# mengxuyiGit/LGM

Measured on AMD Instinct MI355X. Metric: Mpixels/s fwd+bwd Gaussian raster (256^2, 100k gauss, 6 views), higher is better.
Workload: dtype f32

## Files before the change

include/lgm_common.h:

```cpp
#ifndef LGM_COMMON_H
#define LGM_COMMON_H
#include <stddef.h>
#ifdef __cplusplus
extern "C" {
#endif

#define LGM_OK 0
#define LGM_E_INVALID -1
#define LGM_E_WORKSPACE -2
#define LGM_E_HIP -3

const char *lgm_last_error(void);

int lgm_abi_version(void);

typedef struct lgm_profiler lgm_profiler;
lgm_profiler *lgm_profiler_create(void);
int lgm_profiler_summary(lgm_profiler *p, char *buf, size_t len);
int lgm_profiler_reset(lgm_profiler *p);
void lgm_profiler_destroy(lgm_profiler *p);

typedef struct lgm_diag {
    lgm_profiler *profiler;
    unsigned long long *render_counters;
    int det_limit_log2;
} lgm_diag;

#ifdef __cplusplus
}
#endif
#endif
```

lgm_amd/_native.py:

```python
from __future__ import annotations

import contextlib
import ctypes
import os

import torch

LIB_PATH = os.environ.get("LGM_AMD_LIB") or os.path.join(os.path.dirname(os.path.abspath(__file__)), "_lib",
                                                          "liblgm_amd.so")

_c_int, _c_ll, _c_float, _c_size, _vp = ctypes.c_int, ctypes.c_longlong, ctypes.c_float, ctypes.c_size_t, ctypes.c_void_p
_c_double = ctypes.c_double

SIGNATURES = {
    "lgm_abi_version": (_c_int, []),
    "lgm_last_error": (ctypes.c_char_p, []),
    "lgm_render_workspace_size": (_c_size, [_c_int, _c_int, _c_int, _c_int, _c_int, _c_ll]),
    "lgm_render_workspace_size_opts": (_c_size, [_c_int, _c_int, _c_int, _c_int, _c_int, _c_ll, _c_int]),
    "lgm_render_count_pairs": (_c_int, [_c_int, _c_int, _c_int, _c_int, _c_int, _vp, _vp, _vp, _c_float, _c_float,
                                        _c_float, _vp, _c_size, _vp, _vp, _vp]),
    "lgm_render_forward": (_c_int, [_c_int, _c_int, _c_int, _c_int, _c_int, _vp, _vp, _vp, _vp, _c_float, _c_float,
                                    _c_float, _vp, _vp, _vp, _vp, _vp, _c_size, _c_ll, _vp, _c_int, _vp, _vp]),
    "lgm_render_backward": (_c_int, [_c_int, _c_int, _c_int, _c_int, _c_int, _vp, _vp, _vp, _vp, _c_float, _c_float,
                                     _c_float, _vp, _vp, _vp, _vp, _vp, _vp, _c_size, _c_ll, _c_int, _vp, _vp]),
# ... 1 lines not shown
                                  _vp, _vp]),
    "lgm_attn_backward": (_c_int, [_c_int, _c_int, _c_int, _c_int, _c_int, _c_float, _vp, _vp, _vp, _c_ll, _vp, _vp,
                                   _vp, _vp, _vp, _vp, _c_ll, _vp, _c_size, _vp, _vp]),
    "lgm_attn_workspace_size": (_c_size, [_c_int, _c_int, _c_int, _c_int, _c_int]),
    "lgm_mva_workspace_size": (_c_size, [_c_int, _c_int, _c_int, _c_int, _c_int]),
    "lgm_mva_norm_tokens": (_c_int, [_c_int, _c_int, _c_int, _c_int, _c_int, _c_int, _c_int, _c_float, _vp, _vp, _vp,
                                     _vp, _vp, _vp, _vp, _c_size, _vp, _vp]),
    "lgm_mva_tokens_out": (_c_int, [_c_int, _c_int, _c_int, _c_int, _c_int, _c_int, _c_int, _vp, _vp, _c_float, _vp,
                                    _vp, _vp]),
    "lgm_mva_backward_workspace_size": (_c_size, [_c_int, _c_int, _c_int, _c_int, _c_int]),
    "lgm_mva_tokens_out_backward": (_c_int, [_c_int, _c_int, _c_int, _c_int, _c_int, _c_int, _c_int, _vp, _c_float, _vp,
                                             _vp, _vp, _vp]),
    "lgm_mva_norm_tokens_backward": (_c_int, [_c_int, _c_int, _c_int, _c_int, _c_int, _c_int, _c_int, _vp, _vp, _vp,
                                              _vp, _vp, _vp, _vp, _vp, _vp, _vp, _c_size, _vp, _vp]),
    "lgm_render_forward_loss": (_c_int, [_c_int, _c_int, _c_int, _c_int, _c_int, _vp, _vp, _vp, _vp, _c_float,
                                         _c_float, _c_float, _vp, _vp, _vp, _vp, _vp, _vp, _vp, _c_size, _c_ll, _c_int,
                                         _vp, _vp]),
    "lgm_render_backward_loss": (_c_int, [_c_int, _c_int, _c_int, _c_int, _c_int, _vp, _vp, _vp, _vp, _c_float,
                                          _c_float, _c_float, _vp, _vp, _vp, _vp, _vp, _vp, _vp, _c_size, _c_ll,
                                          _c_int, _vp, _vp]),
    "lgm_render_tile_lists": (_c_int, [_c_int, _c_int, _c_int, _c_int, _c_int, _vp, _c_size, _c_ll, _vp, _vp, _vp,
                                       _vp]),
    "lgm_render_pixel_state": (_c_int, [_c_int, _c_int, _c_int, _c_int, _c_int, _vp, _c_size, _c_ll, _vp, _vp, _vp]),
    "lgm_render_records": (_c_int, [_c_int, _c_int, _c_int, _c_int, _c_int, _vp, _c_size, _c_ll, _vp, _vp, _vp, _vp]),
    "lgm_render_needle_flags": (_c_int, [_c_ll, _vp, _vp, _vp]),
    "lgm_render_det_flush_limit_log2": (_c_int, [_c_int, _c_int, _c_int]),
    "lgm_gaussian_head_forward": (_c_int, [_c_int, _c_int, _c_int, _c_int, _c_int, _vp, _vp, _vp, _vp, _vp, _vp,
                                           _c_size, _vp, _vp]),
    "lgm_gaussian_head_workspace_size": (_c_size, [_c_int, _c_int, _c_int, _c_int]),
    "lgm_gaussian_head_backward": (_c_int, [_c_int, _c_int, _c_int, _c_int, _c_int, _vp, _vp, _vp, _vp, _vp, _vp, _vp,
                                            _vp, _vp, _c_size, _vp, _vp]),
    "lgm_linear_wgrad_workspace_size": (_c_size, [_c_int, _c_int, _c_int, _c_int]),
    "lgm_linear_wgrad": (_c_int, [_c_int, _c_int, _c_int, _c_int, _vp, _c_ll, _vp, _c_ll, _vp, _vp, _vp, _c_size,
                                  _vp, _vp]),
    "lgm_conv_wgrad_workspace_size": (_c_size, [_c_int, _c_int, _c_int, _c_int, _c_int, _c_int, _c_int]),
    "lgm_conv_wgrad": (_c_int, [_c_int, _c_int, _c_int, _c_int, _c_int, _c_int, _c_int, _vp, _vp, _vp, _vp, _vp, _c_size,
                                _vp, _vp]),
    "lgm_conv_forward_workspace_size": (_c_size, [_c_int, _c_int, _c_int, _c_int, _c_int, _c_int]),
    "lgm_conv_forward": (_c_int, [_c_int, _c_int, _c_int, _c_int, _c_int, _c_int, _c_int, _c_int, _vp, _vp, _vp, _c_int,
                                  _vp, _vp, _c_size, _vp, _vp]),
    "lgm_conv_dgrad_workspace_size": (_c_size, [_c_int, _c_int, _c_int, _c_int, _c_int, _c_int]),
    "lgm_conv_dgrad": (_c_int, [_c_int, _c_int, _c_int, _c_int, _c_int, _c_int, _c_int, _c_int, _vp, _vp, _vp, _vp,
                                _c_size, _vp, _vp]),
    "lgm_gn_silu_workspace_size": (_c_size, [_c_int, _c_int, _c_int, _c_int, _c_int]),
    "lgm_gn_silu_forward": (_c_int, [_c_int, _c_int, _c_int, _c_int, _c_int, _c_int, _c_int, _c_float, _c_int, _vp, _vp,
                                     _vp, _vp, _vp, _vp, _vp, _c_size, _vp, _vp]),
    "lgm_gn_silu_backward_workspace_size": (_c_size, [_c_int, _c_int, _c_int, _c_int, _c_int]),
    "lgm_gn_silu_backward": (_c_int, [_c_int, _c_int, _c_int, _c_int, _c_int, _c_int, _c_int, _c_int, _vp, _vp, _vp,
                                      _vp, _vp, _vp, _vp, _vp, _vp, _vp, _c_size, _vp, _vp]),
    "lgm_lpips_dist_workspace_size": (_c_size, [_c_int, _c_int, _c_int, _c_int]),
    "lgm_lpips_dist_forward": (_c_int, [_c_int, _c_int, _c_int, _c_int, _c_int, _c_int, _c_float, _vp, _vp, _vp, _vp,
                                        _vp, _vp, _vp, _c_size, _vp, _vp]),
    "lgm_lpips_dist_backward": (_c_int, [_c_int, _c_int, _c_int, _c_int, _c_int, _c_int, _c_float, _vp, _vp, _vp, _vp,
                                         _vp, _vp, _vp, _vp, _vp, _vp]),
    "lgm_lpips_prep_forward": (_c_int, [_c_int, _c_int, _c_int, _c_int, _vp, _vp, _vp, _vp, _vp, _vp, _vp, _vp]),
    "lgm_lpips_prep_backward": (_c_int, [_c_int, _c_int, _c_int, _c_int, _vp, _vp, _vp, _vp]),
    "lgm_data_cameras": (_c_int, [_c_int, _c_int, _c_int, _vp, _vp, _c_double, _c_double, _c_double, _c_double,
                                  _c_double, _vp, _vp, _vp, _vp, _vp, _vp, _vp]),
    "lgm_data_views": (_c_int, [_c_int, _c_int, _c_int, _c_int, _c_int, _c_int, _c_int, _c_int, _c_int, _vp, _vp, _vp,
                                _vp, _c_double, _vp, _vp, _vp, _vp, _vp]),
    "lgm_optim_workspace_size": (_c_size, [_c_ll]),
    "lgm_optim_grad_norm": (_c_int, [_vp, _c_int, _vp, _c_ll, _c_double, _vp, _c_size, _vp, _vp, _vp]),
    "lgm_optim_adamw": (_c_int, [_vp, _c_int, _vp, _c_ll, _c_ll, _vp, _c_double, _c_double, _c_double, _c_double,
                                 _c_double, _c_double, _vp, _vp]),
    "lgm_optim_scale": (_c_int, [_vp, _c_int, _vp, _c_ll, _vp, _vp, _vp]),
    "lgm_mesh_density_workspace_size": (_c_size, [_c_ll, _c_int, _c_int, _c_int, _c_ll]),
    "lgm_mesh_density_count": (_c_int, [_vp, _c_ll, _c_float, _c_int, _c_int, _c_int, _vp, _vp, _c_float, _vp, _c_size,
                                        _vp, _vp, _vp]),
    "lgm_mesh_density": (_c_int, [_vp, _c_ll, _c_float, _c_int, _c_int, _c_int, _vp, _vp, _c_float, _c_ll, _vp, _vp, _vp,
                                  _c_size, _vp, _vp]),
    "lgm_mesh_extract_workspace_size": (_c_size, [_c_int, _c_int, _c_int]),
    "lgm_mesh_count": (_c_int, [_vp, _c_int, _c_int, _c_int, _c_float, _vp, _c_size, _vp, _vp, _vp]),
    "lgm_mesh_emit": (_c_int, [_vp, _vp, _c_int, _c_int, _c_int, _vp, _vp, _c_float, _vp, _c_size, _c_ll, _c_ll, _vp, _vp,
                               _vp, _c_ll, _c_ll, _vp, _vp]),
    "lgm_profiler_create": (_vp, []),
    "lgm_profiler_summary": (_c_int, [_vp, ctypes.c_char_p, _c_size]),
    "lgm_profiler_reset": (_c_int, [_vp]),
    "lgm_profiler_destroy": (None, [_vp]),
}

_lib = None


ABI_VERSION = 10
DTYPE_CODES = {torch.float32: 0, torch.bfloat16: 1, torch.float16: 2}
RENDER_NO_CULL = 1
RENDER_CLAMP_IMAGE = 2
RENDER_BACKWARD_AGAIN = 4
RENDER_DETERMINISTIC = 16
DATA_U8 = 3
OPTIM_CHUNK = 4096


class NativeError(RuntimeError):
    pass


def lib():
    global _lib
    if _lib is None:
        if not os.path.exists(LIB_PATH):
            raise NativeError(f"lgm_amd native library not built ({LIB_PATH}); run `python -m lgm_amd.build`")
        L = ctypes.CDLL(LIB_PATH)
        for name, (res, args) in SIGNATURES.items():
            fn = getattr(L, name, None)
            if fn is None:
                continue
            fn.restype = res
            fn.argtypes = args
        if L.lgm_abi_version() != ABI_VERSION:
            raise NativeError(f"{LIB_PATH}: ABI {L.lgm_abi_version()} != {ABI_VERSION}; rebuild (python -m lgm_amd.build)")
        _lib = L
    return _lib


def check(rc: int, what: str):
    if rc != 0:
        msg = lib().lgm_last_error()
        raise NativeError(f"{what} failed (rc={rc}): {msg.decode() if msg else ''}")


def ptr(t):
    return None if t is None else ctypes.c_void_p(t.data_ptr())


def stream_of(device) -> ctypes.c_void_p:
    return ctypes.c_void_p(torch.cuda.current_stream(device).cuda_stream)


def require_device_tensor(t: torch.Tensor, name: str):
    if not t.is_cuda:
        raise NativeError(f"{name} must be a GPU tensor: lgm_amd has no CPU path (the reference's rasterizer is "
                          "GPU-only too, core/gs.py:20)")


class _Diag(ctypes.Structure):
    _fields_ = [("profiler", _vp), ("render_counters", _vp), ("det_limit_log2", ctypes.c_int)]


_diag_cur = None


def diag():
    return None if _diag_cur is None else ctypes.byref(_diag_cur)


@contextlib.contextmanager
def diagnostics(profiler=None, render_counters=None, det_limit_log2=0):
    global _diag_cur
    prev = _diag_cur
    d = _Diag(profiler.h if profiler is not None else None,
              render_counters.data_ptr() if render_counters is not None else None, int(det_limit_log2))
    _diag_cur = d
    try:
        yield d
    finally:
        _diag_cur = prev


class KernelProfiler:

    def __init__(self):
        self.h = lib().lgm_profiler_create()
        self._cm = None

    def __enter__(self):
        self._cm = diagnostics(profiler=self)
        self._cm.__enter__()
        return self

    def __exit__(self, *exc):
        cm, self._cm = self._cm, None
        return cm.__exit__(*exc)

    def reset(self):
        lib().lgm_profiler_reset(self.h)

    def summary(self):
        buf = ctypes.create_string_buffer(1 << 16)
        check(lib().lgm_profiler_summary(self.h, buf, len(buf)), "lgm_profiler_summary")
        out = {}
        for line in buf.value.decode().splitlines():
            name, n, ms = line.split()
            out[name] = (int(n), float(ms))
        return out

    def close(self):
        if self.h:
            lib().lgm_profiler_destroy(self.h)
            self.h = None
```

lgm_amd/csrc/common.hip:

```cpp
#include "common.h"

#include <stdarg.h>
#include <string.h>

#include <map>
#include <mutex>
#include <string>
#include <vector>

#include "lgm_attn.h"
#include "lgm_common.h"

struct lgm_profiler {
    struct Rec { const char *name; hipEvent_t a, b; };
    std::mutex mu;
    std::vector<Rec> recs;
    std::vector<hipEvent_t> pool;
    size_t used = 0;
    hipEvent_t get() {
        if (used == pool.size()) {
            hipEvent_t e;
            if (hipEventCreate(&e) != hipSuccess) return nullptr;
            pool.push_back(e);
        }
        return pool[used++];
    }
};

namespace lgm {
static thread_local char g_err[512] = {0};
static thread_local const lgm_diag *g_call_diag = nullptr;
static thread_local const char *g_pending = nullptr;
static thread_local hipEvent_t g_pending_ev = nullptr;

void set_error(const char *fmt, ...) {
    va_list ap;
    va_start(ap, fmt);
    vsnprintf(g_err, sizeof(g_err), fmt, ap);
    va_end(ap);
}
void clear_error() { g_err[0] = 0; }

int check_dtype16(const char *who, int dtype) {
    if (dtype == LGM_ATTN_BF16 || dtype == LGM_ATTN_F16) return LGM_OK;
    set_error("%s: dtype must be bf16 or fp16 (got %d)", who, dtype);
    return LGM_E_INVALID;
}
int check_workspace(const char *who, const void *ws, size_t have, size_t need) {
    if (have >= need && (!need || ws)) return LGM_OK;
    set_error("%s: workspace too small (%zu < %zu bytes)", who, ws ? have : 0, need);
    return LGM_E_WORKSPACE;
}

static thread_local int g_scope_depth = 0;
DiagScope::DiagScope(const lgm_diag *d) {
    if (g_scope_depth++ == 0) g_call_diag = d;
}
DiagScope::~DiagScope() {
    if (--g_scope_depth == 0) {
        g_call_diag = nullptr;
        g_pending_ev = nullptr;
    }
}
const lgm_diag *call_diag() { return g_call_diag; }

static lgm_profiler *call_profiler() { return g_call_diag ? g_call_diag->profiler : nullptr; }

void prof_begin(const char *name, hipStream_t st) {
    lgm_profiler *p = call_profiler();
    if (!p) return;
    std::lock_guard<std::mutex> lk(p->mu);
    g_pending = name;
    g_pending_ev = p->get();
    if (g_pending_ev) (void)hipEventRecord(g_pending_ev, st);
}
void prof_end(hipStream_t st) {
    lgm_profiler *p = call_profiler();
    if (!p || !g_pending_ev) return;
    std::lock_guard<std::mutex> lk(p->mu);
    hipEvent_t b = p->get();
    if (!b) return;
    (void)hipEventRecord(b, st);
    p->recs.push_back({g_pending, g_pending_ev, b});
    g_pending_ev = nullptr;
}
}

extern "C" {
const char *lgm_last_error(void) { return lgm::g_err; }
int lgm_abi_version(void) { return 10; }

lgm_profiler *lgm_profiler_create(void) { return new lgm_profiler(); }
int lgm_profiler_reset(lgm_profiler *p) {
    if (!p) return LGM_E_INVALID;
    std::lock_guard<std::mutex> lk(p->mu);
    p->recs.clear();
    p->used = 0;
    return LGM_OK;
}
int lgm_profiler_summary(lgm_profiler *p, char *buf, size_t len) {
    if (!p || !buf || len == 0) return LGM_E_INVALID;
    std::map<std::string, std::pair<int, double>> agg;
    std::vector<std::string> order;
    for (auto &r : p->recs) {
        if (hipEventSynchronize(r.b) != hipSuccess) {
            lgm::set_error("event sync failed");
            return LGM_E_HIP;
        }
        float ms = 0.f;
        (void)hipEventElapsedTime(&ms, r.a, r.b);
        auto it = agg.find(r.name);
        if (it == agg.end()) {
            order.push_back(r.name);
            agg[r.name] = {1, ms};
        } else {
            it->second.first++;
            it->second.second += ms;
        }
    }
    std::string out;
    char line[256];
    for (auto &n : order) {
        snprintf(line, sizeof(line), "%s %d %.6f\n", n.c_str(), agg[n].first, agg[n].second);
        out += line;
    }
    strncpy(buf, out.c_str(), len - 1);
    buf[len - 1] = 0;
    return LGM_OK;
}
void lgm_profiler_destroy(lgm_profiler *p) {
    if (!p) return;
    for (auto e : p->pool) (void)hipEventDestroy(e);
    delete p;
}
}
```

lgm_amd/csrc/render_bin.hip:

```cpp
#include "render_common.h"

namespace lgm {
namespace {

enum BinMode { COUNT = 0, EMIT_SLOT = 1, EMIT_PACKED = 2 };

template <int CTRL, int ROW_MASK = 0xf>
__device__ __forceinline__ int dpp_src(int old, int v) {
    return __builtin_amdgcn_update_dpp(old, v, CTRL, ROW_MASK, 0xf, false);
}
__device__ __forceinline__ int wave_incl_scan(int x, int ) {
    x += dpp_src<0x111>(0, x);
    x += dpp_src<0x112>(0, x);
    x += dpp_src<0x114>(0, x);
    x += dpp_src<0x118>(0, x);
    x += dpp_src<0x142, 0xa>(0, x);
    x += dpp_src<0x143, 0xc>(0, x);
    return x;
}

constexpr int BIN_THREADS = 512, BIN_G = BIN_THREADS, BIN_ITERS = 3;
constexpr int BIN_HITCAP = BIN_THREADS * 6;
static_assert(BIN_THREADS <= 512, "owner index and tile rank pack into 9 bits each");
static_assert(LDS_HIST_MAX <= 1 << 13, "the tile index of a hit packs into 13 bits");
#ifndef LGM_BIN_WAVES
#define LGM_BIN_WAVES 6
#endif
constexpr int bin_waves(bool stats) { return stats ? 4 : LGM_BIN_WAVES; }

struct BinRec {
    float x, y, kB, k0, k1, dys, mg;
    unsigned c0;
    unsigned cx1;
    unsigned pad_;
    unsigned long long key;
};

__device__ __forceinline__ int wave_incl_max(int v, int ) {
    constexpr int LO = -2147483647 - 1;
    v = max(v, dpp_src<0x111>(LO, v));
    v = max(v, dpp_src<0x112>(LO, v));
    v = max(v, dpp_src<0x114>(LO, v));
    v = max(v, dpp_src<0x118>(LO, v));
    v = max(v, dpp_src<0x142, 0xa>(LO, v));
    v = max(v, dpp_src<0x143, 0xc>(LO, v));
    return v;
}

__device__ void center_order(int gx, int T, int *__restrict__ corder, int *hk) {
    const int gy = (T + gx - 1) / gx, tid = threadIdx.x, w = tid >> 6, lane = tid & 63;
    const int K = min(T, BIN_THREADS);
    const long long maxkey = (long long)(gx - 1) * (gx - 1) + (long long)(gy - 1) * (gy - 1);
    auto key = [&](int t) {
        const int y = t / gx, x = t - y * gx, dx = 2 * x - (gx - 1), dy = 2 * y - (gy - 1);
        return maxkey ? (int)(((long long)dx * dx + (long long)dy * dy) * (K - 1) / maxkey) : 0;
    };
    __syncthreads();
    if (tid < K) hk[tid] = 0;
    __syncthreads();
    for (int t = tid; t < T; t += BIN_THREADS) atomicAdd(&hk[key(t)], 1);
    __syncthreads();
    const int v = tid < K ? hk[tid] : 0;
    const int incl = wave_incl_scan(v, lane);
    if (lane == 63) hk[K + w] = incl;
    __syncthreads();
    int run = incl - v;
    for (int ww = 0; ww < w; ww++) run += hk[K + ww];
    __syncthreads();
    if (tid < K) hk[tid] = run;
    __syncthreads();
    for (int t = tid; t < T; t += BIN_THREADS) corder[atomicAdd(&hk[key(t)], 1)] = t;
}

template <int MODE, bool STATS, bool STAMPS>
__global__ __launch_bounds__(BIN_THREADS) __attribute__((amdgpu_waves_per_eu(bin_waves(STATS)))) void k_bin(
    Dims d, const float *__restrict__ gauss, const float *__restrict__ views, const float *__restrict__ projs,
    float4 *__restrict__ gP, float4 *__restrict__ gQ, uint2 *__restrict__ rects, int *__restrict__ radii_out,
    int *__restrict__ tile_count, const int *__restrict__ tile_start, unsigned long long *__restrict__ pairs,
    long long slot_stride, unsigned long long *__restrict__ misc, float *__restrict__ accum,
    int *__restrict__ corder) {
    extern __shared__ int hist[];
    __shared__ BinRec srec[BIN_THREADS];
    __shared__ int sHead[BIN_THREADS], sExcl[BIN_THREADS];
    __shared__ unsigned sHit[BIN_HITCAP];
    __shared__ int s_nhit;
    __shared__ unsigned long long s_tot[2];
    const int T = d.T, tid = threadIdx.x, w = tid >> 6, lane = tid & 63;
    const int vgroups = (d.V + BIN_ITERS - 1) / BIN_ITERS;
    const int b = blockIdx.y / vgroups, vg0 = (blockIdx.y - b * vgroups) * BIN_ITERS;
    int bv = b * d.V + vg0;
    const bool lds = T <= LDS_HIST_MAX;
    int *hbase = hist + T, *fill = hist + 2 * T;
    int *cur = tile_count + (size_t)bv * T;
    if constexpr (STATS)
        if (tid < 2) s_tot[tid] = 0;
    auto dest = [&](int t, int pos) -> long long {
        return (MODE == EMIT_SLOT ? ((long long)bv * T + t) * slot_stride
                                  : (long long)tile_start[(size_t)bv * T + t]) + pos;
    };
    __shared__ unsigned long long s_ph[4];
    unsigned long long *stamp = nullptr;
    if constexpr (STAMPS) {
        stamp = d.counters + 8 + 8 * (size_t)d.BV * T + 8 * ((size_t)blockIdx.y * gridDim.x + blockIdx.x);
        if (tid == 0) {
            s_ph[0] = s_ph[1] = s_ph[2] = 0;
            stamp[0] = s_ph[3] = __builtin_amdgcn_s_memrealtime();
        }
    }
    auto phase = [&](int k) {
        if constexpr (STAMPS) {
            if (tid == 0) {
                const unsigned long long t = __builtin_amdgcn_s_memrealtime();
                if (k >= 0) s_ph[k] += t - s_ph[3];
                s_ph[3] = t;
            }
        }
    };
    const int i = blockIdx.x * BIN_G + tid;
    float c3[6];
    if (i < d.N) {
        float g[14];
        load_gaussian(gauss + ((size_t)b * d.N + i) * 14, g);
        gaussian_cov3d(g, d.mod, c3);
    }
    for (int it = 0; it < BIN_ITERS; it++) {
    if (vg0 + it >= d.V) break;
    bv = b * d.V + vg0 + it;
    cur = tile_count + (size_t)bv * T;
    if (tid == 0) s_nhit = 0;
    if (lds)
        for (int t = tid; t < T; t += BIN_THREADS) hist[t] = 0;
    Geo o;
    bool vis = false;
    if (i < d.N) {
        const float2 *gp = reinterpret_cast<const float2 *>(gauss + ((size_t)b * d.N + i) * 14);
        const float2 g01 = gp[0], g23 = gp[1];
        const float gm[4] = {g01.x, g01.y, g23.x, g23.y};
        vis = preprocess_view(gm, c3, views + 16 * bv, projs + 16 * bv, d, o);
        if (MODE != COUNT) {
            const size_t k = (size_t)bv * d.N + i;
            if (vis) {
                const float4 rp = rec_p(o.x, o.y, o.A, o.B), rq = rec_q(o.C, o.opacity, o.tau, o.depth);
                gP[k] = rp;
                gQ[k] = rq;
                const bool side = !(d.options & LGM_RENDER_DETERMINISTIC) && rec_needle(rp.z, rp.w, rq.x);
                rects[k] = make_uint2((unsigned)o.x0 | ((unsigned)o.y0 << 16),
                                      (unsigned)o.x1 | ((unsigned)o.y1 << 16) | (side ? 0x80000000u : 0u));
                if (side) {
                    double *sd = reinterpret_cast<double *>(accum + acc_side_offset(d.B, d.V, d.N)) + k * 3;
                    sd[0] = 0.0; sd[1] = 0.0; sd[2] = 0.0;
                }
            } else {
                gP[k] = make_float4(0.f, 0.f, 0.f, 0.f);
                gQ[k] = make_float4(0.f, -INFINITY, -1.f, 0.f);
                rects[k] = make_uint2(0u, 0u);
            }
            if (radii_out) radii_out[k] = vis ? o.radius : 0;
        }
    }
    int nc = 0;
    unsigned long long nref = 0;
    if (vis) {
        BinRec r;
        r.x = o.x; r.y = o.y;
        const float detq = o.A * o.C - o.B * o.B;
        if (o.tau >= 3.0e38f || !(detq > 0.f) || !(o.A > 0.f) || !(o.C > 0.f)) {
            r.kB = 0.f; r.k0 = INFINITY; r.k1 = 0.f; r.dys = 0.f; r.mg = 0.f;
        } else {
            const float iA = __builtin_amdgcn_rcpf(o.A);
            r.kB = o.B * iA;
            r.k0 = fmaxf(o.tau, 0.f) * iA;
            r.k1 = detq * iA * iA;
            const float hxe = sqrtf(fmaxf(o.tau, 0.f) * o.C * __builtin_amdgcn_rcpf(detq));
            r.dys = -o.B * hxe * __builtin_amdgcn_rcpf(o.C);
            r.mg = 1e-3f * hxe + 1e-2f;
        }
        r.c0 = (unsigned)o.cx0 | ((unsigned)o.cy0 << 16);
        r.cx1 = (unsigned)o.cx1;
        r.key = ((unsigned long long)__float_as_uint(o.depth) << 32) | (unsigned)i;
        srec[tid] = r;
        nc = o.cx1 > o.cx0 ? o.cy1 - o.cy0 : 0;
        if constexpr (STATS) nref = (unsigned long long)((o.x1 - o.x0) * (o.y1 - o.y0));
    }
    if constexpr (STATS) {
#pragma unroll
        for (int o2 = 32; o2 > 0; o2 >>= 1) nref += __shfl_xor(nref, o2, 64);
        if (lane == 0 && nref) atomicAdd(&s_tot[1], nref);
    }
    const int incl = wave_incl_scan(nc, lane), excl = incl - nc;
    const int total = __builtin_amdgcn_readlane(incl, 63);
    sExcl[tid] = excl;
    __syncthreads();
    phase(0);
    unsigned long long nemit = 0;
    auto flat_tests = [&](int pass) {
    int carry = 0;
    for (int base0 = 0; base0 < total; base0 += 64) {
        sHead[tid] = -1;
        __builtin_amdgcn_fence(__ATOMIC_RELEASE, "wavefront");
        if (nc > 0 && excl >= base0 && excl < base0 + 64) sHead[w * 64 + excl - base0] = lane;
        __builtin_amdgcn_fence(__ATOMIC_ACQ_REL, "wavefront");
        int v = sHead[tid];
        if (lane == 0 && v < 0) v = carry;
        v = wave_incl_max(v, lane);
        carry = __builtin_amdgcn_readlane(v, 63);
        const int c = base0 + lane;
        int ta = 0, cnt = 0, trow = 0, owner = 0;
        if (c < total) {
            owner = w * 64 + v;
            const BinRec &e = srec[owner];
            const int ty = (int)(e.c0 >> 16) + (c - sExcl[owner]);
            const float dy0 = (float)(ty * BY) - e.y, dy1 = dy0 + (float)(BY - 1);
            const float e1 = fminf(fmaxf(e.dys, dy0), dy1), e2 = fminf(fmaxf(-e.dys, dy0), dy1);
            const float xh = e.x - e.kB * e1 + sqrtf(fmaxf(e.k0 - e.k1 * e1 * e1, 0.f)) + e.mg;
            const float xl = e.x - e.kB * e2 - sqrtf(fmaxf(e.k0 - e.k1 * e2 * e2, 0.f)) - e.mg;
            const int cx0 = (int)(e.c0 & 0xffffu), cx1 = (int)e.cx1;
            const float fa = ceilf((xl - (float)(BX - 1)) * (1.0f / BX)), fb = floorf(xh * (1.0f / BX)) + 1.f;
            ta = (int)fminf(fmaxf(fa, (float)cx0), (float)cx1);
            const int tb = (int)fminf(fmaxf(fb, (float)ta), (float)cx1);
            cnt = tb - ta;
            trow = ty * d.gx;
        }
        if (pass == 1) {
            for (int k = 0; k < cnt; k++) {
                const int t = trow + ta + k;
                pairs[dest(t, hbase[t] + atomicAdd(&fill[t], 1))] = srec[owner].key;
            }
            continue;
        }
        const int hincl = wave_incl_scan(cnt, lane);
        const int htot = __builtin_amdgcn_readlane(hincl, 63);
        if constexpr (STATS) nemit += (unsigned)htot;
        if (!htot) continue;
        if (lds) {
            int slot0 = 0;
            if (MODE != COUNT && lane == 0) slot0 = atomicAdd(&s_nhit, htot);
            slot0 = __builtin_amdgcn_readlane(slot0, 0) + hincl - cnt;
            for (int k = 0; k < cnt; k++) {
                const int t = trow + ta + k;
                const int rk = atomicAdd(&hist[t], 1);
                if (MODE != COUNT) {
                    const int slot = slot0 + k;
                    if (slot < BIN_HITCAP) sHit[slot] = (unsigned)owner | ((unsigned)rk << 9) | ((unsigned)t << 18);
                }
            }
        } else {
            for (int k = 0; k < cnt; k++) {
                const int t = trow + ta + k;
                const int pos = atomicAdd(&cur[t], 1);
                if (MODE != COUNT) pairs[dest(t, pos)] = srec[owner].key;
            }
        }
    }
    };
    flat_tests(0);
    if constexpr (STATS)
        if (lane == 0 && nemit) atomicAdd(&s_tot[0], nemit);
    if (lds) {
        __syncthreads();
        phase(1);
        for (int t = tid; t < T; t += BIN_THREADS) {
            const int c = hist[t];
            if (c) {
                if (MODE == COUNT) atomicAdd(&cur[t], c);
                else hbase[t] = atomicAdd(&cur[t], c);
            }
            fill[t] = 0;
        }
        __syncthreads();
        phase(2);
        if (MODE != COUNT) {
            const int H = s_nhit;
            if (H <= BIN_HITCAP) {
                for (int h = tid; h < H; h += BIN_THREADS) {
                    const unsigned e2 = sHit[h];
                    const int t = (int)(e2 >> 18);
                    pairs[dest(t, hbase[t] + (int)((e2 >> 9) & 511u))] = srec[e2 & 511u].key;
                }
            } else {
                flat_tests(1);
            }
        }
    }
    __syncthreads();
    phase(-1);
    if (STAMPS && tid == 0) {
        stamp[1] = s_ph[0];
        stamp[2] = s_ph[1];
        stamp[3] = s_ph[2];
        stamp[4] = s_ph[3];
        stamp[5] = (unsigned long long)s_nhit;
        stamp[6] = __builtin_amdgcn_s_getreg((31 << 11) | 4);
        stamp[7] = __builtin_amdgcn_s_getreg((3 << 11) | 20);
    }
    }
    if (STATS && tid == 0) {
        atomicAdd(&misc[0], s_tot[0]);
        atomicAdd(&misc[1], s_tot[1]);
    }
    if (corder && blockIdx.x == 0 && blockIdx.y == 0) center_order(d.gx, T, corder, hist);
}

template <int MODE>
auto bin_kernel(bool stats, bool stamps) {
    return stats ? (stamps ? k_bin<MODE, true, true> : k_bin<MODE, true, false>)
                 : (stamps ? k_bin<MODE, false, true> : k_bin<MODE, false, false>);
}

__global__ __launch_bounds__(1024) void k_scan(const int *__restrict__ count, int M, int *__restrict__ start) {
    __shared__ long long wsum[16];
    const int tid = threadIdx.x, lane = tid & 63, wid = tid >> 6;
    const int per = (M + 1023) / 1024;
    const int lo = min(M, tid * per), hi = min(M, lo + per);
    long long s = 0;
    for (int i = lo; i < hi; i++) s += count[i];
    long long x = s;
#pragma unroll
    for (int dd = 1; dd < 64; dd <<= 1) {
        const long long y = __shfl_up(x, dd, 64);
        if (lane >= dd) x += y;
    }
    if (lane == 63) wsum[wid] = x;
    __syncthreads();
    if (wid == 0) {
        long long w = lane < 16 ? wsum[lane] : 0;
#pragma unroll
        for (int dd = 1; dd < 16; dd <<= 1) {
            const long long y = __shfl_up(w, dd, 64);
            if (lane >= dd) w += y;
        }
        if (lane < 16) wsum[lane] = w;
    }
    __syncthreads();
    long long run = x - s + (wid > 0 ? wsum[wid - 1] : 0);
    for (int i = lo; i < hi; i++) {
        start[i] = (int)run;
        run += count[i];
    }
    if (tid == 1023) start[M] = (int)wsum[15];
}

constexpr int RS_THREADS = 512, RS_WAVES = RS_THREADS / 64, RS_CAP = 4032,
              RS_MAXR = (RS_CAP + RS_THREADS - 1) / RS_THREADS;
constexpr int RS_OBLK = 4096;
static_assert(RS_CAP <= RS_OBLK && RS_CAP % 64 == 0, "sort image layout");
constexpr int RS_DBITS = 9, RS_B = 1 << RS_DBITS;
typedef unsigned short RsCnt;
constexpr int RS_LDS_LSD = RS_CAP * 4 + RS_CAP * 2 + RS_WAVES * RS_B * (int)sizeof(RsCnt);
constexpr int RS_LDS = RS_LDS_LSD > RS_CAP * 8 + 2048 * 4 ? RS_LDS_LSD : RS_CAP * 8 + 2048 * 4;
static_assert(RS_CAP < 65536, "u16 counters");
static_assert(RS_LDS >= RS_OBLK * 8, "sort_oversized reuses the image as u64[RS_OBLK]");
static_assert(RS_LDS + 512 <= 160 * 1024 / 4, "4 sort workgroups per CU (with the static __shared__ words)");
static_assert(RS_B % RS_THREADS == 0 || RS_THREADS % RS_B == 0, "bucket scan layout");

__device__ __forceinline__ unsigned long long lanemask_lt(int lane) { return (1ull << lane) - 1ull; }

__device__ __forceinline__ unsigned long long match_digit(unsigned dgt, bool valid, int nbits) {
    unsigned long long peers = __ballot(valid);
    for (int b = 0; b < nbits; b++) {
        const bool bit = (dgt >> b) & 1u;
        const unsigned long long m = __ballot(bit);
        peers &= bit ? m : ~m;
    }
    return peers;
}

__device__ __forceinline__ unsigned wave_min_u32(unsigned v) {
#pragma unroll
    for (int o = 32; o > 0; o >>= 1) v = min(v, (unsigned)__shfl_xor((int)v, o, 64));
    return v;
}
__device__ __forceinline__ unsigned wave_max_u32(unsigned v) {
#pragma unroll
    for (int o = 32; o > 0; o >>= 1) v = max(v, (unsigned)__shfl_xor((int)v, o, 64));
    return v;
}

__device__ __forceinline__ void radix_pass(const unsigned (&kr)[RS_MAXR], const unsigned short (&pr)[RS_MAXR],
                                          int shift, int nbits, int n, int c0, int R, unsigned *sk,
                                          unsigned short *sp, RsCnt *cnt, int *s_wsum) {
    const int tid = threadIdx.x, w = tid >> 6, lane = tid & 63;
    const unsigned mask = (1u << nbits) - 1u;
    RsCnt *my = cnt + w * RS_B;
// ... 305 lines not shown
            const int e = c0 + r * 64 + lane;
            if (r < R && e < n) idr[r] = (unsigned)seg[sp[e]];
        }
        bool any_tie = false;
        for (int q = tid; q + 1 < n; q += RS_THREADS) any_tie |= sk[q] == sk[q + 1];
        if (__syncthreads_or(any_tie)) {
            unsigned *ids_l = reinterpret_cast<unsigned *>(sp);
#pragma unroll
            for (int r = 0; r < RS_MAXR; r++) {
                const int e = c0 + r * 64 + lane;
                if (r < R && e < n) ids_l[e] = idr[r];
            }
            __syncthreads();
            for (int q = tid; q < n; q += RS_THREADS) {
                if (q + 1 < n && sk[q] == sk[q + 1] && (q == 0 || sk[q - 1] != sk[q])) {
                    int e = q + 1;
                    while (e < n && sk[e] == sk[q]) e++;
                    for (int a2 = q + 1; a2 < e; a2++) {
                        const unsigned v = ids_l[a2];
                        int z = a2 - 1;
                        while (z >= q && ids_l[z] > v) { ids_l[z + 1] = ids_l[z]; z--; }
                        ids_l[z + 1] = v;
                    }
                }
            }
            __syncthreads();
#pragma unroll
            for (int r = 0; r < RS_MAXR; r++) {
                const int e = c0 + r * 64 + lane;
                if (r < R && e < n) idr[r] = ids_l[e];
            }
        }
    }
    __syncthreads();
    unsigned *ids = reinterpret_cast<unsigned *>(seg);
#pragma unroll
    for (int r = 0; r < RS_MAXR; r++) {
        const int e = c0 + r * 64 + lane;
        if (r < R && e < n) ids[e] = idr[r];
    }
}

__global__ __launch_bounds__(RS_THREADS) __attribute__((amdgpu_waves_per_eu(8))) void k_sort(
    int M, long long slot_stride, const int *__restrict__ tile_start, const int *__restrict__ tile_count,
    unsigned long long *__restrict__ pairs, unsigned long long *__restrict__ counters, int BV, int T,
    const int *__restrict__ corder) {
    int tile = xcd_item(blockIdx.x, M);
    if (corder) {
        const int r = (int)blockIdx.x / BV, v = (int)blockIdx.x - r * BV;
        tile = v * T + corder[r];
    }
    long long base;
    int n;
    tile_range(tile, slot_stride, tile_start, tile_count, base, n);
    const unsigned long long t_start = __builtin_amdgcn_s_memrealtime();
    if (counters && threadIdx.x == 0) {
        counters[8 + 8 * (size_t)tile + 4] = t_start;
        counters[8 + 8 * (size_t)tile + 6] = (unsigned long long)n;
    }
    sort_tile(base, n, pairs);
    if (counters) {
        __syncthreads();
        if (threadIdx.x == 0) counters[8 + 8 * (size_t)tile + 5] = __builtin_amdgcn_s_memrealtime();
    }
}

}

int launch_binning(const Dims &d, const float *gaussians, const float *cam_view, const float *cam_view_proj,
                   char *ws, const Layout &L, int *radii_out, long long *stats_out, bool count_only,
                   hipStream_t st) {
    const size_t M = (size_t)d.BV * d.T;
    if (hipMemsetAsync(ws + L.tile_count, 0, L.misc + 64 - L.tile_count, st) != hipSuccess) {
        set_error("hipMemsetAsync failed");
        return LGM_E_HIP;
    }
    float4 *gP = (float4 *)(ws + L.gP), *gQ = (float4 *)(ws + L.gQ);
    uint2 *rects = (uint2 *)(ws + L.rects);
    int *tcount = (int *)(ws + L.tile_count), *tstart = (int *)(ws + L.tile_start);
    unsigned long long *pairs = (unsigned long long *)(ws + L.pairs), *misc = (unsigned long long *)(ws + L.misc);
    float *accum = (float *)(ws + L.accum);
    const size_t lds = d.T <= LDS_HIST_MAX ? 3 * (size_t)d.T * 4 : 0;
    int *corder = lds && d.T >= 8 ? (int *)(ws + L.order) : nullptr;
    dim3 grid((d.N + BIN_G - 1) / BIN_G, d.B * ((d.V + BIN_ITERS - 1) / BIN_ITERS));
    const bool stats = stats_out != nullptr || count_only, stamps = d.counters != nullptr;
    if (d.N > 0) {
        if (count_only || !L.slot) {
            LGM_LAUNCH("k_bin_count", st, (bin_kernel<COUNT>(stats, stamps)<<<grid, BIN_THREADS, lds, st>>>(
                       d, gaussians, cam_view, cam_view_proj, gP, gQ, rects, nullptr, tcount, tstart, pairs, 0, misc,
                       accum, nullptr)));
        }
        if (!count_only) {
            if (L.slot) {
                LGM_LAUNCH("k_bin", st, (bin_kernel<EMIT_SLOT>(stats, stamps)<<<grid, BIN_THREADS, lds, st>>>(
                           d, gaussians, cam_view, cam_view_proj, gP, gQ, rects, radii_out, tcount, tstart, pairs,
                           (long long)d.N, misc, accum, corder)));
            } else {
                LGM_LAUNCH("k_scan", st, (k_scan<<<1, 1024, 0, st>>>(tcount, (int)M, tstart)));
                if (hipMemsetAsync(ws + L.tile_count, 0, L.misc + 64 - L.tile_count, st) != hipSuccess) {
                    set_error("hipMemsetAsync failed");
                    return LGM_E_HIP;
                }
                LGM_LAUNCH("k_bin", st, (bin_kernel<EMIT_PACKED>(stats, stamps)<<<grid, BIN_THREADS, lds, st>>>(
                           d, gaussians, cam_view, cam_view_proj, gP, gQ, rects, radii_out, tcount, tstart, pairs, 0,
                           misc, accum, corder)));
            }
            LGM_LAUNCH("k_sort", st, (k_sort<<<(unsigned)M, RS_THREADS, RS_LDS, st>>>(
                                         (int)M, L.slot ? (long long)d.N : -1LL, tstart, tcount, pairs, d.counters,
                                         d.BV, d.T, corder)));
        }
    }
    if (d.N == 0 && !L.slot && hipMemsetAsync(ws + L.tile_start, 0, (M + 1) * 4, st) != hipSuccess) {
        set_error("hipMemsetAsync failed");
        return LGM_E_HIP;
    }
    if (stats_out && hipMemcpyAsync(stats_out, ws + L.misc, 16, hipMemcpyDeviceToDevice, st) != hipSuccess) {
        set_error("hipMemcpyAsync failed");
        return LGM_E_HIP;
    }
    return LGM_OK;
}

}
```

lgm_amd/csrc/render_common.h:

```cpp
#pragma once
#include <hip/hip_runtime.h>
#include <stdint.h>

#include "common.h"
#include "lgm_render.h"
#include "work_split.h"

namespace lgm {

constexpr int BX = 16, BY = 16, TILE_PIX = BX * BY;
constexpr int NACC = 10;
constexpr int NACC_V = 6, NACC_S = 4;
__host__ __device__ __forceinline__ size_t acc_index(int q, size_t bvN_i, size_t bN_i, size_t BVN) {
    return q < 5 ? bvN_i * NACC_V + q : q < 9 ? BVN * NACC_V + bN_i * NACC_S + (q - 5) : bvN_i * NACC_V + 5;
}
__host__ __device__ inline size_t acc_elems(size_t B, size_t V, size_t N) { return B * V * N * NACC_V + B * N * NACC_S; }
__host__ __device__ inline size_t acc_side_offset(size_t B, size_t V, size_t N) { return (acc_elems(B, V, N) + 1) & ~(size_t)1; }
__host__ __device__ inline int det_flush_limit_log2(int V, int T, bool scene_record) {
    const long long f = scene_record ? (long long)V * T : (long long)T;
    int c = 0;
    while ((1ll << c) < f) c++;
    return 62 - c;
}
constexpr int LDS_HIST_MAX = 8192;
constexpr float LOG2E = 1.4426950408889634f;

inline size_t align_up(size_t x) { return (x + 255) & ~size_t(255); }
constexpr float ACC_NEEDLE = 300.0f;

struct Layout {
    size_t gP, gQ, rects, tile_count, tile_start, order, pairs, final_T, n_contrib, wlast, cfin, ck, cklist, nck, cmask,
        accum, lossp, lossw, detmax, misc, total;
    long long cap;
    int ck_region;
    int ck_slots;
    bool slot;
};

#ifndef LGM_CK_LONG_TILES
#define LGM_CK_LONG_TILES 4096
#endif
constexpr size_t CK_LONG_TILES = LGM_CK_LONG_TILES;
#ifdef LGM_CK_SHIFT0
__host__ __device__ __forceinline__ int ck_shift_for(size_t) { return 0; }
#else
__host__ __device__ __forceinline__ int ck_shift_for(size_t tiles) { return tiles >= CK_LONG_TILES ? 1 : 0; }
#endif

inline Layout make_layout(int B, int V, int N, int H, int W, long long pair_capacity, bool det = false) {
    const size_t BV = (size_t)B * V, T = (size_t)((W + BX - 1) / BX) * ((H + BY - 1) / BY), P = (size_t)H * W;
    Layout L;
    L.slot = pair_capacity <= 0;
    L.cap = L.slot ? (long long)(BV * T * (size_t)N) : pair_capacity;
    size_t o = 0;
    auto take = [&](size_t bytes) { size_t r = o; o = align_up(o + bytes); return r; };
    L.gP = take(BV * N * 16);
    L.gQ = take(BV * N * 16);
    L.rects = take(BV * N * 8);
    L.tile_count = take(BV * T * 4);
    L.misc = take(64);
    L.tile_start = take((BV * T + 1) * 4);
    L.order = take(T * 4);
    L.pairs = take((size_t)L.cap * 8);
    L.final_T = take(BV * P * 4);
    L.n_contrib = take(BV * P * 4);
    L.wlast = take(BV * T * 16);
    L.cfin = take(BV * P * 16);
    L.ck_region = (int)std::min((2 * BV * T + 7) / 8, ((3 * BV * T / 4) >> ck_shift_for(BV * T)) / 8 + 1 + 256);
    L.ck_slots = det ? 0 : 8 * L.ck_region;
    L.ck = take((size_t)L.ck_slots * 5 * TILE_PIX * 4);
    L.cklist = take((size_t)L.ck_slots * 8);
    L.nck = take(BV * T * 4);
    L.cmask = take(BV * P);
    L.accum = take(det ? acc_elems(B, V, N) * 8 : acc_side_offset(B, V, N) * 4 + BV * N * 3 * 8);
    L.lossp = take(BV * T * 2 * 4);
    L.lossw = take(((BV * T + 2047) / 2048) * 16);
    L.detmax = take(64 * 4);
    L.total = o;
    return L;
}

struct Dims {
    int B, V, N, H, W, gx, gy, T, BV;
    float tanx, tany, fx, fy, mod;
    unsigned long long *counters;
    int det_lim_log2;
    int options;
    int ck_shift;
    const float *gt_img, *gt_mask;
    float *loss_part;
    float *loss_out;
    const float *d_loss;
};

__device__ __forceinline__ void xf43(const float *M, float x, float y, float z, float o[3]) {
#pragma clang fp contract(off)
    o[0] = M[0] * x + M[4] * y + M[8] * z + M[12];
    o[1] = M[1] * x + M[5] * y + M[9] * z + M[13];
    o[2] = M[2] * x + M[6] * y + M[10] * z + M[14];
}
__device__ __forceinline__ void xf44(const float *M, float x, float y, float z, float o[4]) {
#pragma clang fp contract(off)
    o[0] = M[0] * x + M[4] * y + M[8] * z + M[12];
    o[1] = M[1] * x + M[5] * y + M[9] * z + M[13];
    o[2] = M[2] * x + M[6] * y + M[10] * z + M[14];
    o[3] = M[3] * x + M[7] * y + M[11] * z + M[15];
}

__device__ __forceinline__ void quat_rot(const float q[4], float R[3][3]) {
#pragma clang fp contract(off)
    const float r = q[0], x = q[1], y = q[2], z = q[3];
    R[0][0] = 1.f - 2.f * (y * y + z * z); R[0][1] = 2.f * (x * y - r * z); R[0][2] = 2.f * (x * z + r * y);
    R[1][0] = 2.f * (x * y + r * z); R[1][1] = 1.f - 2.f * (x * x + z * z); R[1][2] = 2.f * (y * z - r * x);
    R[2][0] = 2.f * (x * z - r * y); R[2][1] = 2.f * (y * z + r * x); R[2][2] = 1.f - 2.f * (x * x + y * y);
}

__device__ __forceinline__ void cov3d(const float s[3], const float R[3][3], float c3[6]) {
#pragma clang fp contract(off)
    float M[3][3];
#pragma unroll
    for (int c = 0; c < 3; c++)
#pragma unroll
        for (int k = 0; k < 3; k++) M[c][k] = s[k] * R[c][k];
#define LGM_SIG(c, r) (M[r][0] * M[c][0] + M[r][1] * M[c][1] + M[r][2] * M[c][2])
    c3[0] = LGM_SIG(0, 0); c3[1] = LGM_SIG(0, 1); c3[2] = LGM_SIG(0, 2);
    c3[3] = LGM_SIG(1, 1); c3[4] = LGM_SIG(1, 2); c3[5] = LGM_SIG(2, 2);
#undef LGM_SIG
}

struct ProjCtx {
    float T0[3], T1[3];
    float t[3];
    float xmul, ymul;
};
__device__ __forceinline__ ProjCtx make_proj(const float *Vw, float mx, float my, float mz, float fx, float fy,
                                             float tanx, float tany) {
#pragma clang fp contract(off)
    ProjCtx P;
    xf43(Vw, mx, my, mz, P.t);
    const float limx = 1.3f * tanx, limy = 1.3f * tany;
    const float txtz = P.t[0] / P.t[2], tytz = P.t[1] / P.t[2];
    P.t[0] = fminf(limx, fmaxf(-limx, txtz)) * P.t[2];
    P.t[1] = fminf(limy, fmaxf(-limy, tytz)) * P.t[2];
    P.xmul = (txtz < -limx || txtz > limx) ? 0.f : 1.f;
    P.ymul = (tytz < -limy || tytz > limy) ? 0.f : 1.f;
    const float tz = P.t[2];
    const float J00 = fx / tz, J02 = -(fx * P.t[0]) / (tz * tz);
    const float J11 = fy / tz, J12 = -(fy * P.t[1]) / (tz * tz);
#pragma unroll
    for (int r = 0; r < 3; r++) {
        P.T0[r] = Vw[4 * r + 0] * J00 + Vw[4 * r + 2] * J02;
        P.T1[r] = Vw[4 * r + 1] * J11 + Vw[4 * r + 2] * J12;
    }
    return P;
}
__device__ __forceinline__ void cov2d(const ProjCtx &P, const float c3[6], float &a, float &b, float &c) {
#pragma clang fp contract(off)
    const float S[3][3] = {{c3[0], c3[1], c3[2]}, {c3[1], c3[3], c3[4]}, {c3[2], c3[4], c3[5]}};
    float s0[3], s1[3];
#pragma unroll
    for (int k = 0; k < 3; k++) {
        s0[k] = S[k][0] * P.T0[0] + S[k][1] * P.T0[1] + S[k][2] * P.T0[2];
// ... 179 lines not shown
```

Before: 2624.

## Plan binning workgroup shape per CU occupancy with views-per-unit and tail split

Replaces the fixed 2D binning grid (gaussian blocks × view groups of 3) with a 1D grid driven by a host-side plan. The plan picks how many views each workgroup handles (1 to 3) and optionally splits the last partial wave into single-view units, using CU count, LDS and wave occupancy and a linear cost model. The goal is to cut wave-quantization tail imbalance in the binning kernel. It adds host queries of the device attribute per call and a heuristic cost model that may mispredict.

```diff
diff --git a/include/lgm_common.h b/include/lgm_common.h
--- a/include/lgm_common.h
+++ b/include/lgm_common.h
@@ -24,6 +24,8 @@
     lgm_profiler *profiler;
     unsigned long long *render_counters;
     int det_limit_log2;
+    int bin_views;
+    int bin_slots;
 } lgm_diag;
 
 #ifdef __cplusplus
diff --git a/lgm_amd/_native.py b/lgm_amd/_native.py
--- a/lgm_amd/_native.py
+++ b/lgm_amd/_native.py
@@ -107,7 +107,7 @@
 _lib = None
 
 
-ABI_VERSION = 10
+ABI_VERSION = 11
 DTYPE_CODES = {torch.float32: 0, torch.bfloat16: 1, torch.float16: 2}
 RENDER_NO_CULL = 1
 RENDER_CLAMP_IMAGE = 2
@@ -160,7 +160,8 @@
 
 
 class _Diag(ctypes.Structure):
-    _fields_ = [("profiler", _vp), ("render_counters", _vp), ("det_limit_log2", ctypes.c_int)]
+    _fields_ = [("profiler", _vp), ("render_counters", _vp), ("det_limit_log2", ctypes.c_int),
+                ("bin_views", ctypes.c_int), ("bin_slots", ctypes.c_int)]
 
 
 _diag_cur = None
@@ -171,11 +172,12 @@
 
 
 @contextlib.contextmanager
-def diagnostics(profiler=None, render_counters=None, det_limit_log2=0):
+def diagnostics(profiler=None, render_counters=None, det_limit_log2=0, bin_views=0, bin_slots=0):
     global _diag_cur
     prev = _diag_cur
     d = _Diag(profiler.h if profiler is not None else None,
-              render_counters.data_ptr() if render_counters is not None else None, int(det_limit_log2))
+              render_counters.data_ptr() if render_counters is not None else None, int(det_limit_log2),
+              int(bin_views), int(bin_slots))
     _diag_cur = d
     try:
         yield d
diff --git a/lgm_amd/csrc/common.hip b/lgm_amd/csrc/common.hip
--- a/lgm_amd/csrc/common.hip
+++ b/lgm_amd/csrc/common.hip
@@ -88,7 +88,7 @@
 
 extern "C" {
 const char *lgm_last_error(void) { return lgm::g_err; }
-int lgm_abi_version(void) { return 10; }
+int lgm_abi_version(void) { return 11; }
 
 lgm_profiler *lgm_profiler_create(void) { return new lgm_profiler(); }
 int lgm_profiler_reset(lgm_profiler *p) {
diff --git a/lgm_amd/csrc/render_bin.hip b/lgm_amd/csrc/render_bin.hip
--- a/lgm_amd/csrc/render_bin.hip
+++ b/lgm_amd/csrc/render_bin.hip
@@ -27,6 +27,7 @@
 #define LGM_BIN_WAVES 6
 #endif
 constexpr int bin_waves(bool stats) { return stats ? 4 : LGM_BIN_WAVES; }
+static_assert(BIN_ITERS == 3, "plan_binning prices and bounds the views of a unit as 1..3");
 
 struct BinRec {
     float x, y, kB, k0, k1, dys, mg;
@@ -35,6 +36,8 @@
     unsigned pad_;
     unsigned long long key;
 };
+constexpr size_t BIN_STATIC_LDS = sizeof(BinRec) * BIN_THREADS + 2 * 4 * BIN_THREADS + 4 * BIN_HITCAP + 56;
+constexpr size_t CU_LDS_BYTES = 160 * 1024;
 
 __device__ __forceinline__ int wave_incl_max(int v, int ) {
     constexpr int LO = -2147483647 - 1;
@@ -78,7 +81,7 @@
     float4 *__restrict__ gP, float4 *__restrict__ gQ, uint2 *__restrict__ rects, int *__restrict__ radii_out,
     int *__restrict__ tile_count, const int *__restrict__ tile_start, unsigned long long *__restrict__ pairs,
     long long slot_stride, unsigned long long *__restrict__ misc, float *__restrict__ accum,
-    int *__restrict__ corder) {
+    int *__restrict__ corder, BinPlan pl) {
     extern __shared__ int hist[];
     __shared__ BinRec srec[BIN_THREADS];
     __shared__ int sHead[BIN_THREADS], sExcl[BIN_THREADS];
@@ -86,9 +89,9 @@
     __shared__ int s_nhit;
     __shared__ unsigned long long s_tot[2];
     const int T = d.T, tid = threadIdx.x, w = tid >> 6, lane = tid & 63;
-    const int vgroups = (d.V + BIN_ITERS - 1) / BIN_ITERS;
-    const int b = blockIdx.y / vgroups, vg0 = (blockIdx.y - b * vgroups) * BIN_ITERS;
-    int bv = b * d.V + vg0;
+    const BinUnit un = bin_unit(pl, d.V, (int)blockIdx.x);
+    const int b = un.row / d.V;
+    int bv = un.row;
     const bool lds = T <= LDS_HIST_MAX;
     int *hbase = hist + T, *fill = hist + 2 * T;
     int *cur = tile_count + (size_t)bv * T;
@@ -101,7 +104,7 @@
     __shared__ unsigned long long s_ph[4];
     unsigned long long *stamp = nullptr;
     if constexpr (STAMPS) {
-        stamp = d.counters + 8 + 8 * (size_t)d.BV * T + 8 * ((size_t)blockIdx.y * gridDim.x + blockIdx.x);
+        stamp = d.counters + 8 + 8 * (size_t)d.BV * T + 8 * (size_t)blockIdx.x;
         if (tid == 0) {
             s_ph[0] = s_ph[1] = s_ph[2] = 0;
             stamp[0] = s_ph[3] = __builtin_amdgcn_s_memrealtime();
@@ -116,7 +119,7 @@
             }
         }
     };
-    const int i = blockIdx.x * BIN_G + tid;
+    const int i = un.x * BIN_G + tid;
     float c3[6];
     if (i < d.N) {
         float g[14];
@@ -124,8 +127,8 @@
         gaussian_cov3d(g, d.mod, c3);
     }
     for (int it = 0; it < BIN_ITERS; it++) {
-    if (vg0 + it >= d.V) break;
-    bv = b * d.V + vg0 + it;
+    if (it >= un.nv) break;
+    bv = un.row + it;
     cur = tile_count + (size_t)bv * T;
     if (tid == 0) s_nhit = 0;
     if (lds)
@@ -289,7 +292,7 @@
         stamp[2] = s_ph[1];
         stamp[3] = s_ph[2];
         stamp[4] = s_ph[3];
-        stamp[5] = (unsigned long long)s_nhit;
+        stamp[5] = (unsigned long long)s_nhit | ((unsigned long long)un.nv << 32);
         stamp[6] = __builtin_amdgcn_s_getreg((31 << 11) | 4);
         stamp[7] = __builtin_amdgcn_s_getreg((3 << 11) | 20);
     }
@@ -298,7 +301,7 @@
         atomicAdd(&misc[0], s_tot[0]);
         atomicAdd(&misc[1], s_tot[1]);
     }
-    if (corder && blockIdx.x == 0 && blockIdx.y == 0) center_order(d.gx, T, corder, hist);
+    if (corder && blockIdx.x == 0) center_order(d.gx, T, corder, hist);
 }
 
 template <int MODE>
@@ -770,19 +773,40 @@
     float *accum = (float *)(ws + L.accum);
     const size_t lds = d.T <= LDS_HIST_MAX ? 3 * (size_t)d.T * 4 : 0;
     int *corder = lds && d.T >= 8 ? (int *)(ws + L.order) : nullptr;
-    dim3 grid((d.N + BIN_G - 1) / BIN_G, d.B * ((d.V + BIN_ITERS - 1) / BIN_ITERS));
     const bool stats = stats_out != nullptr || count_only, stamps = d.counters != nullptr;
+    const int blocks = (d.N + BIN_G - 1) / BIN_G;
+    if ((long long)d.BV * blocks > 0x7fffffffLL) {
+        set_error("too many binning workgroups (B=%d V=%d N=%d)", d.B, d.V, d.N);
+        return LGM_E_INVALID;
+    }
+    const lgm_diag *diag = call_diag();
+    long long slots = diag ? diag->bin_slots : 0;
+    int per_cu = 1;
+    if (slots <= 0) {
+        int dev = 0, cus = 0;
+        if (hipGetDevice(&dev) != hipSuccess ||
+            hipDeviceGetAttribute(&cus, hipDeviceAttributeMultiprocessorCount, dev) != hipSuccess) {
+            set_error("hipDeviceGetAttribute failed");
+            return LGM_E_HIP;
+        }
+        const int by_waves = bin_waves(stats) * 4 * 64 / BIN_THREADS;
+        const int by_lds = (int)(CU_LDS_BYTES / (BIN_STATIC_LDS + lds));
+        per_cu = std::max(1, std::min(by_waves, by_lds));
+        slots = (long long)cus * per_cu;
+    }
+    const BinPlan pl = plan_binning(blocks, d.B, d.V, slots, per_cu, diag ? diag->bin_views : 0);
+    const dim3 grid((unsigned)(pl.main_wg + pl.tail_wg));
     if (d.N > 0) {
         if (count_only || !L.slot) {
             LGM_LAUNCH("k_bin_count", st, (bin_kernel<COUNT>(stats, stamps)<<<grid, BIN_THREADS, lds, st>>>(
                        d, gaussians, cam_view, cam_view_proj, gP, gQ, rects, nullptr, tcount, tstart, pairs, 0, misc,
-                       accum, nullptr)));
+                       accum, nullptr, pl)));
         }
         if (!count_only) {
             if (L.slot) {
                 LGM_LAUNCH("k_bin", st, (bin_kernel<EMIT_SLOT>(stats, stamps)<<<grid, BIN_THREADS, lds, st>>>(
                            d, gaussians, cam_view, cam_view_proj, gP, gQ, rects, radii_out, tcount, tstart, pairs,
-                           (long long)d.N, misc, accum, corder)));
+                           (long long)d.N, misc, accum, corder, pl)));
             } else {
                 LGM_LAUNCH("k_scan", st, (k_scan<<<1, 1024, 0, st>>>(tcount, (int)M, tstart)));
                 if (hipMemsetAsync(ws + L.tile_count, 0, L.misc + 64 - L.tile_count, st) != hipSuccess) {
@@ -791,7 +815,7 @@
                 }
                 LGM_LAUNCH("k_bin", st, (bin_kernel<EMIT_PACKED>(stats, stamps)<<<grid, BIN_THREADS, lds, st>>>(
                            d, gaussians, cam_view, cam_view_proj, gP, gQ, rects, radii_out, tcount, tstart, pairs, 0,
-                           misc, accum, corder)));
+                           misc, accum, corder, pl)));
             }
             LGM_LAUNCH("k_sort", st, (k_sort<<<(unsigned)M, RS_THREADS, RS_LDS, st>>>(
                                          (int)M, L.slot ? (long long)d.N : -1LL, tstart, tcount, pairs, d.counters,
diff --git a/lgm_amd/csrc/render_common.h b/lgm_amd/csrc/render_common.h
--- a/lgm_amd/csrc/render_common.h
+++ b/lgm_amd/csrc/render_common.h
@@ -78,6 +78,77 @@
     L.detmax = take(64 * 4);
     L.total = o;
     return L;
+}
+
+struct BinPlan {
+    int v, vgroups, blocks;
+    int main_wg, tail_wg;
+    int tail_part, x0, row0, row1;
+};
+struct BinUnit {
+    int x, row, nv;
+};
+__host__ __device__ __forceinline__ BinUnit bin_unit(const BinPlan &p, int V, int u) {
+    BinUnit r;
+    if (u < p.main_wg) {
+        const int y = u / p.blocks, b = y / p.vgroups, first = (y - b * p.vgroups) * p.v;
+        r.x = u - y * p.blocks;
+        r.row = b * V + first;
+        r.nv = V - first < p.v ? V - first : p.v;
+        return r;
+    }
+    int t = u - p.main_wg;
+    r.nv = 1;
+    if (t < p.tail_part) {
+        const int w0 = p.blocks - p.x0, it = t / w0;
+        r.x = p.x0 + t - it * w0;
+        r.row = p.row0 + it;
+    } else {
+        t -= p.tail_part;
+        const int q = t / p.blocks;
+        r.x = t - q * p.blocks;
+        r.row = p.row1 + q;
+    }
+    return r;
+}
+constexpr float BIN_C0 = -1.8f, BIN_C1 = 11.9f;
+inline float bin_chain_cost(int v) { return BIN_C0 + (float)v * BIN_C1; }
+inline BinPlan bin_shape(int blocks, int B, int V, int v, long long slots, bool split) {
+    BinPlan p;
+    p.v = v;
+    p.vgroups = (V + v - 1) / v;
+    p.blocks = blocks;
+    const long long W = (long long)B * p.vgroups * blocks;
+    p.main_wg = (int)W;
+    p.tail_wg = p.tail_part = p.x0 = p.row0 = p.row1 = 0;
+    const long long r = slots > 0 ? W % slots : 0;
+    if (!split || slots <= 0 || W <= slots || r == 0 || r * v > slots) return p;
+    p.main_wg = (int)(W - r);
+    const int y0 = p.main_wg / blocks, b0 = y0 / p.vgroups, vg0 = y0 - b0 * p.vgroups;
+    p.x0 = p.main_wg - y0 * blocks;
+    p.row0 = b0 * V + vg0 * v;
+    p.row1 = vg0 + 1 < p.vgroups ? p.row0 + v : (b0 + 1) * V;
+    p.tail_part = (p.row1 - p.row0) * (blocks - p.x0);
+    p.tail_wg = p.tail_part + (B * V - p.row1) * blocks;
+    return p;
+}
+inline float bin_plan_cost(const BinPlan &p, long long slots) {
+    if (slots <= 0) return bin_chain_cost(p.v);
+    const long long full = p.main_wg / slots, r = p.main_wg % slots;
+    return (float)(full + (r ? 1 : 0)) * bin_chain_cost(p.v) + (p.tail_wg ? bin_chain_cost(1) : 0.f);
+}
+inline BinPlan plan_binning(int blocks, int B, int V, long long slots, int per_cu, int force_v = 0) {
+    if (force_v >= 1 && force_v <= 3) return bin_shape(blocks, B, V, force_v, slots, true);
+    BinPlan best = bin_shape(blocks, B, V, 3, slots, false);
+    if (per_cu < 3 || (long long)best.main_wg * per_cu <= slots) return best;
+    float cb = bin_plan_cost(best, slots);
+    for (int v = 3; v >= 1; v--)
+        for (int split = 0; split < 2; split++) {
+            const BinPlan p = bin_shape(blocks, B, V, v, slots, split != 0);
+            const float c = bin_plan_cost(p, slots);
+            if (c < cb) { best = p; cb = c; }
+        }
+    return best;
 }
 
 struct Dims {
```

New measurement: 2634 (median of 6 runs). Within noise of the previous version (+0.4%).
